# gitouni/Spatial-Temporal-LiDAR-camera-Calibration

Hardware: NVIDIA B200
Metric: extrinsic_cost_evals_per_s (higher is better)
Workload: dtype f64

## Files before the change

### include/stlcalib.h

```cpp
#ifndef STLCALIB_H_
#define STLCALIB_H_

#include <stdint.h>

#ifdef __cplusplus
extern "C" {
#endif

#define STL_ABI_VERSION 2
#define STL_MAX_COVIS 10

typedef enum stl_status {
    STL_OK = 0,
    STL_ERR_INVALID = 1,
    STL_ERR_CUDA = 2,
    STL_ERR_NO_DEVICE = 3,
    STL_ERR_STATE = 4,
    STL_ERR_CAPACITY = 5
} stl_status_t;

typedef struct stl_params {
    double max_pixel_dist;
    double corr_3d_2d_threshold;
    double corr_3d_3d_threshold;
// ... 171 lines not shown

stl_status_t stl_select_keyframes(stl_ctx_t *ctx, const int32_t *kf, int32_t n);

stl_status_t stl_eval_frames(stl_ctx_t *ctx, const double *x, int32_t B, double *out);


stl_status_t stl_debug_corrset(stl_ctx_t *ctx, int32_t b, int32_t kf, uint32_t *kp_idx,
                               uint32_t *pt_idx, int32_t cap, int32_t *n);

stl_status_t stl_debug_align(stl_ctx_t *ctx, int32_t b, int32_t kf, uint32_t *kp_idx,
                             uint32_t *nn_idx, int32_t *n_neigh, int32_t *is_plane, double *dist,
                             uint32_t *knn_idx, int32_t cap, int32_t *n);

stl_status_t stl_debug_frame(stl_ctx_t *ctx, int32_t b, int32_t kf, double out[13]);

stl_status_t stl_knn3d(stl_ctx_t *ctx, int32_t kf, const double *q, int32_t nq, int32_t k,
                       double radius2, uint32_t *out_idx, double *out_d2, int32_t *out_count);

stl_status_t stl_debug_trig(stl_ctx_t *ctx, const double *x, int32_t n, double *acos_out, double *cos_out);


#define STL_STAGE_ASSOC2D 0
#define STL_STAGE_KNN3D 1
#define STL_STAGE_REDUCE 2
#define STL_STAGE_LINEARIZE 3
#define STL_STAGE_BUILD 4
#define STL_STAGE_ASSOC_LM 5
#define STL_STAGE_ALLREDUCE 6
#define STL_STAGE_PLANE_INDEX 7
#define STL_NSTAGES 8
// ... 13 lines not shown
```

### spatial-temporal-lidar-camera-calibration_b200/_abi.py

```python
from __future__ import annotations

import ctypes as C
import os

_HERE = os.path.dirname(os.path.abspath(__file__))

STL_MAX_COVIS = 10
STL_EVAL_NSUMS = 12
STL_LIN_NSUMS = 62
STL_STEP_NSUMS = STL_EVAL_NSUMS + STL_LIN_NSUMS
STL_COMM_ID_BYTES = 128
STL_MAX_PROBLEMS = 256
STL_NSTAGES = 8
STAGE_NAMES = ("assoc2d", "knn3d", "reduce", "linearize", "build", "assoc_lm", "allreduce", "plane_index")

STATUS = {0: "STL_OK", 1: "STL_ERR_INVALID", 2: "STL_ERR_CUDA", 3: "STL_ERR_NO_DEVICE",
          4: "STL_ERR_STATE", 5: "STL_ERR_CAPACITY"}


class StlError(RuntimeError):
    def __init__(self, code: int, msg: str = ""):
        self.code = code
        super().__init__(f"{STATUS.get(code, code)}: {msg}")

# ... 87 lines not shown
        ("width", C.c_int32), ("height", C.c_int32),
        ("fx", C.c_float), ("fy", C.c_float), ("cx", C.c_float), ("cy", C.c_float),
        ("anchored_frac", C.c_double), ("mappoint_frac", C.c_double), ("match_frac", C.c_double),
        ("outlier_frac", C.c_double), ("scale_gt", C.c_double), ("kf_spacing", C.c_double),
        ("max_range", C.c_double), ("elev_top_deg", C.c_double), ("elev_bottom_deg", C.c_double),
        ("x_gt", C.c_double * 7), ("seed", C.c_uint64),
    ]


_vp = C.c_void_p
_dp = C.POINTER(C.c_double)
_u32p = C.POINTER(C.c_uint32)
_i32p = C.POINTER(C.c_int32)
_i64p = C.POINTER(C.c_int64)
_u8p = C.POINTER(C.c_uint8)

CALIB_SYMBOLS = {
    "stl_default_params": (None, [C.POINTER(Params)]),
    "stl_create": (C.c_int, [C.POINTER(Params), C.c_int32, C.POINTER(_vp)]),
    "stl_destroy": (None, [_vp]),
    "stl_last_error": (C.c_char_p, [_vp]),
    "stl_abi_version": (C.c_int32, []),
    "stl_upload_pack": (C.c_int, [_vp, C.POINTER(Pack)]),
    "stl_eval_batch": (C.c_int, [_vp, _dp, C.c_int32, C.POINTER(EvalSums)]),
    "stl_eval_batch_device": (C.c_int, [_vp, _dp, C.c_int32, _vp, _vp]),
    "stl_finalize": (None, [C.POINTER(Params), C.POINTER(EvalSums), C.POINTER(BAErrorOut)]),
    "stl_bbo": (None, [C.POINTER(Params), C.POINTER(BAErrorOut), _dp]),
    "stl_associate": (C.c_int, [_vp, _dp, _i64p]),
    "stl_linearize_batch": (C.c_int, [_vp, _dp, C.c_int32, C.POINTER(LinSums)]),
    "stl_linearize_batch_device": (C.c_int, [_vp, _dp, C.c_int32, _vp, _vp]),
# ... 12 lines not shown
    "stl_step_multi_device": (C.c_int, [_vp, _dp, C.c_int32, _u8p, _vp, _vp]),
    "stl_he_linearize": (C.c_int, [_vp, C.POINTER(HeEdges), _dp, C.c_int32, C.POINTER(LinSums), _dp]),
    "stl_calib_linearize": (C.c_int, [_vp, C.POINTER(CalibEdges), _dp, C.c_int32, C.POINTER(LinSums), _dp]),
    "stl_comm_unique_id": (C.c_int, [C.POINTER(C.c_uint8)]),
    "stl_comm_init": (C.c_int, [_vp, C.POINTER(C.c_uint8), C.c_int32, C.c_int32]),
    "stl_comm_info": (C.c_int, [_vp, _i32p, _i32p]),
    "stl_comm_stats": (C.c_int, [_vp, _i64p]),
    "stl_select_keyframes": (C.c_int, [_vp, _i32p, C.c_int32]),
    "stl_eval_frames": (C.c_int, [_vp, _dp, C.c_int32, _dp]),
    "stl_allow_oversize_keyframes": (C.c_int, [_vp, C.c_int32]),
    "stl_oversize_keyframes": (C.c_int, [_vp, _i32p, C.c_int32, _i32p]),
    "stl_debug_corrset": (C.c_int, [_vp, C.c_int32, C.c_int32, _u32p, _u32p, C.c_int32, _i32p]),
    "stl_debug_align": (C.c_int, [_vp, C.c_int32, C.c_int32, _u32p, _u32p, _i32p, _i32p, _dp, _u32p,
                                  C.c_int32, _i32p]),
    "stl_debug_frame": (C.c_int, [_vp, C.c_int32, C.c_int32, _dp]),
    "stl_debug_trig": (C.c_int, [_vp, _dp, C.c_int32, _dp, _dp]),
    "stl_knn3d": (C.c_int, [_vp, C.c_int32, _dp, C.c_int32, C.c_int32, C.c_double, _u32p, _dp, _i32p]),
    "stl_set_stream": (C.c_int, [_vp, _vp]),
    "stl_set_profiling": (C.c_int, [_vp, C.c_int32]),
    "stl_stage_stats": (C.c_int, [_vp, _dp, _i64p]),
    "stl_work_counters": (C.c_int, [_vp, _dp]),
}

SYNTH_SYMBOLS = {
    "stl_synth_default_cfg": (None, [C.POINTER(SynthCfg)]),
    "stl_synth_create": (_vp, [C.POINTER(SynthCfg)]),
    "stl_synth_pack": (C.POINTER(Pack), [_vp]),
    "stl_synth_x_gt": (_dp, [_vp]),
    "stl_synth_Twl": (_dp, [_vp]),
    "stl_synth_destroy": (None, [_vp]),
# ... 38 lines not shown
```

### spatial-temporal-lidar-camera-calibration_b200/capi.py

```python
from __future__ import annotations

import ctypes as C

import numpy as np

from . import _abi
from .pack import KeyFramePack, default_params

_dp = _abi._dp


def _check(lib, h, code):
    if code != 0:
        msg = lib.stl_last_error(h).decode() if h else ""
        raise _abi.StlError(code, msg)


class Context:

    def __init__(self, params: _abi.Params | None = None, device: int = 0):
        self.lib = _abi.load_calib()
        self.params = params if params is not None else default_params()
        h = C.c_void_p()
        code = self.lib.stl_create(C.byref(self.params), device, C.byref(h))
# ... 294 lines not shown
        knn = np.zeros((cap, 32), np.uint32)
        n = C.c_int32(0)
        _check(self.lib, self.h, self.lib.stl_debug_align(
            self.h, b, kf, kp.ctypes.data_as(_abi._u32p), nn.ctypes.data_as(_abi._u32p), m.ctypes.data_as(_abi._i32p),
            pl.ctypes.data_as(_abi._i32p), d.ctypes.data_as(_dp), knn.ctypes.data_as(_abi._u32p), cap, C.byref(n)))
        k = n.value
        return dict(kp=kp[:k], nn=nn[:k], m=m[:k], is_plane=pl[:k], dist=d[:k], knn=knn[:k])

    def debug_frame(self, b: int, kf: int):
        out = np.zeros(13)
        _check(self.lib, self.h, self.lib.stl_debug_frame(self.h, b, kf, out.ctypes.data_as(_dp)))
        names = ("sum_3d2d", "valid_3d2d", "cnt_3d2d", "sum_he", "cnt_he", "kept", "n_corr", "n_queries",
                 "sum_3d3d", "valid_3d3d", "cnt_3d3d", "valid_pl", "valid_pt")
        return dict(zip(names, out))

    def debug_trig(self, x):
        x = np.ascontiguousarray(x, dtype=np.float64).reshape(-1)
        a, c = np.zeros_like(x), np.zeros_like(x)
        _check(self.lib, self.h, self.lib.stl_debug_trig(self.h, x.ctypes.data_as(_dp), len(x), a.ctypes.data_as(_dp), c.ctypes.data_as(_dp)))
        return a, c

    def knn3d(self, kf: int, q, k: int, radius2: float = 0.0):
        q = np.ascontiguousarray(q, dtype=np.float64).reshape(-1, 3)
        nq = q.shape[0]
        idx = np.zeros((nq, k), np.uint32)
        d2 = np.zeros((nq, k), np.float64)
        cnt = np.zeros(nq, np.int32)
        _check(self.lib, self.h, self.lib.stl_knn3d(self.h, kf, q.ctypes.data_as(_dp), nq, k, radius2,
                                                    idx.ctypes.data_as(_abi._u32p), d2.ctypes.data_as(_dp),
                                                    cnt.ctypes.data_as(_abi._i32p)))
# ... 80 lines not shown
```

### spatial-temporal-lidar-camera-calibration_b200/csrc/capi.cu

```cuda
#include <algorithm>
#include <cfloat>
#include <climits>
#include <cmath>
#include <cstdarg>
#include <cstdio>
#include <cstdlib>
#include <cstring>
#include <mutex>
#include <string>
#include <vector>

#include <nccl.h>

#include "../../include/stlcalib.h"
#include "gprfit.hpp"
#include "hostmath.hpp"
#include "kernels.h"
#include "lm.h"
#include "packlayout.hpp"

using namespace stl;

struct stl_ctx {
    int device = 0;
// ... 82 lines not shown
    }
    return st;
}

#define CK(call)                                                                                          \
    do {                                                                                                  \
        cudaError_t e_ = (call);                                                                          \
        if (e_ != cudaSuccess) return fail(ctx, STL_ERR_CUDA, "%s: %s (%s:%d)", #call, cudaGetErrorString(e_), __FILE__, __LINE__); \
    } while (0)

template <class T> void dfree(T *&p) { if (p) { cudaFree(p); p = nullptr; } }

void free_pack(stl_ctx *c) {
    DevPack &p = c->pk;
    dfree(p.kf); dfree(p.px); dfree(p.py); dfree(p.pz); dfree(p.orig); dfree(p.node_lo); dfree(p.node_hi); dfree(p.adj); dfree(p.adj_cov);
    dfree(p.pl_rec); dfree(p.pl_m);
    dfree(p.k1tab); dfree(p.bitmap); dfree(p.grid_start); dfree(p.grid_kp); dfree(p.kp_xy); dfree(p.kp_xyd); dfree(p.kp_mp); dfree(p.Tcw);
    dfree(p.relpose); dfree(p.covis_valid); dfree(p.covis_uv); dfree(p.he_Tc); dfree(p.he_Tl);
    p = DevPack();
    dfree(c->d_frames); dfree(c->d_ov);
    for (stl_ctx::DevRoute *d : {&c->d_all, &c->d_sel}) { dfree(d->lists); dfree(d->sel); dfree(d->sel_mp); *d = stl_ctx::DevRoute(); }
    c->lay = PackLayout();
    c->route = KfRoute();
    c->has_pack = false;
}
void free_work(stl_ctx *c) {
    DevWork &w = c->wk;
    dfree(w.cand); dfree(w.corr_kp); dfree(w.corr_pt); dfree(w.corr_sp); dfree(w.q_corr); dfree(w.q_kpsp); dfree(w.n_corr); dfree(w.n_q);
    dfree(w.k1_ticket); dfree(w.k1_rec); dfree(w.k1_match); dfree(w.k1_ov_match); dfree(w.k1_surv); dfree(w.k1_cnt); dfree(w.k1_best_d2); dfree(w.k1_best_key);
    dfree(w.frame); dfree(w.align); dfree(w.nn_pos); dfree(w.nn_g2); dfree(w.nb); dfree(w.nbx); dfree(w.nb_m); dfree(w.nb_last); dfree(w.dbg_nn); dfree(w.dbg_m); dfree(w.dbg_plane); dfree(w.dbg_dist); dfree(w.dbg_knn); dfree(w.dbg_stats);
    dfree(w.overflow); dfree(w.k1_clk);
// ... 537 lines not shown
            CK(cudaMemcpy(row.data(), pk.adj + hk[f].node_off * 32, row.size() * 2, cudaMemcpyDeviceToHost));
            cov.resize((size_t)nl);
            CK(cudaMemcpy(cov.data(), pk.adj_cov + hk[f].node_off, cov.size() * 4, cudaMemcpyDeviceToHost));
            for (int l = 0; l < nl; ++l) if (cov[l] >= 0 && cov[l] < 1e30f) { ++partial; cov_sum += std::sqrt((double)cov[l]); }
            for (int l = 0; l < nl; ++l) {
                int c = 0;
                for (int t = 0; t < 32; ++t) c += row[(size_t)l * 32 + t] != 0xffffu;
                ++real; empty += c == 0; entries += c;
            }
        }
        fprintf(stderr, "[stl] leaf adjacency (sampled keyframes): %lld leaves, %.2f%% without a row, %.1f neighbours per row, %.1f%% truncated (mean coverage %.3f m)\n", real,
                100.0 * empty / std::max<long long>(real, 1), (double)entries / std::max<long long>(real - empty, 1),
                100.0 * partial / std::max<long long>(real, 1), cov_sum / std::max<long long>(partial, 1));
    }
    if (ctx->params.plane_index) {
        CK(cudaMalloc(&pk.pl_rec, sizeof(PlaneRec) * npt));
        CK(cudaMalloc(&pk.pl_m, 4 * npt));
        CK(cudaEventRecord(ev0, st));
        for (int f0 = 0; f0 < F;) {
            int f1 = f0 + 1;
            long long pts = hk[f0].n_pad;
            while (f1 < F && pts + hk[f1].n_pad <= (4ll << 20)) pts += hk[f1++].n_pad;
            cudaError_t e = build_plane_index(pk, hk.data(), f0, f1 - f0, ctx->dpr, st, scope.scr);
            if (e != cudaSuccess) return fail(ctx, STL_ERR_CUDA, "plane index: %s", cudaGetErrorString(e));
            f0 = f1;
        }
        CK(cudaEventRecord(ev1, st));
        CK(cudaStreamSynchronize(st));
        float ms = 0;
        CK(cudaEventElapsedTime(&ms, ev0, ev1));
        ctx->stage_ms[STL_STAGE_PLANE_INDEX] += ms;
        ctx->stage_n[STL_STAGE_PLANE_INDEX] += 1;
// ... 85 lines not shown
    if (m <= 0) return STL_OK;
    const long long off = ctx->lay.kf[kf].kp_off;
    if (kp_idx) {
        int nc = 0;
        CK(cudaMemcpy(&nc, ctx->wk.n_corr + kf, 4, cudaMemcpyDeviceToHost));
        std::vector<uint32_t> qc(m), ck(std::max(nc, 1));
        CK(cudaMemcpy(qc.data(), ctx->wk.q_corr + off, 4 * (size_t)m, cudaMemcpyDeviceToHost));
        CK(cudaMemcpy(ck.data(), ctx->wk.corr_kp + off, 4 * (size_t)nc, cudaMemcpyDeviceToHost));
        for (int i = 0; i < m; ++i) kp_idx[i] = ck[qc[i]];
    }
    if (nn_idx) CK(cudaMemcpy(nn_idx, ctx->wk.dbg_nn + off, 4 * (size_t)m, cudaMemcpyDeviceToHost));
    if (n_neigh) CK(cudaMemcpy(n_neigh, ctx->wk.dbg_m + off, 4 * (size_t)m, cudaMemcpyDeviceToHost));
    if (is_plane) CK(cudaMemcpy(is_plane, ctx->wk.dbg_plane + off, 4 * (size_t)m, cudaMemcpyDeviceToHost));
    if (dist) CK(cudaMemcpy(dist, ctx->wk.dbg_dist + off, 8 * (size_t)m, cudaMemcpyDeviceToHost));
    if (knn_idx) CK(cudaMemcpy(knn_idx, ctx->wk.dbg_knn + off * kMaxK, 4 * (size_t)m * kMaxK, cudaMemcpyDeviceToHost));
    return STL_OK;
}

stl_status_t stl_debug_frame(stl_ctx_t *ctx, int32_t b, int32_t kf, double out[13]) {
    if (!ctx || !out) return STL_ERR_INVALID;
    std::lock_guard<std::mutex> lk(ctx->mu);
    CK(cudaSetDevice(ctx->device));
    stl_status_t s = run_debug(ctx, b);
    if (s != STL_OK) return s;
    if (kf < 0 || kf >= ctx->pk.n_kf) return fail(ctx, STL_ERR_INVALID, "keyframe out of range");
    if (!kf_selected(ctx, kf)) { for (int i = 0; i < 13; ++i) out[i] = 0; return STL_OK; }
    FrameRec r;
    CK(cudaMemcpy(&r, ctx->wk.frame + kf, sizeof(r), cudaMemcpyDeviceToHost));
    std::vector<AlignRec> a(ctx->wk.sub);
    CK(cudaMemcpy(a.data(), ctx->wk.align + (size_t)kf * ctx->wk.sub, sizeof(AlignRec) * ctx->wk.sub, cudaMemcpyDeviceToHost));
// ... 645 lines not shown
```

### spatial-temporal-lidar-camera-calibration_b200/csrc/common.cuh

```cuda
#pragma once
#include <cstdint>
#include <cuda_runtime.h>

namespace stl {

constexpr int kLeaf = 32;
constexpr int kPadPts = 128;
constexpr int kBmCell = 2;
constexpr int kGridCell = 8;
constexpr float kFastErrPx = 0.25f;
constexpr int kMaxK = 32;

struct DevKf {
    long long pt_off;
    long long node_off;
    long long kp_off;
    long long bm_off;
    long long grid_off;
    long long mp_off;
    long long tab_off;
    int n_mp;
    int tab_bytes;
    int n_pts, n_pad;
    int n0, n1, n2;
// ... 25 lines not shown
    double s;
    float sf;
    float pad_;
};

struct FrameRec {
    double s2d, v2d, c2d;
    double she, che;
    double kept, ncorr;
    double nq;
};
struct AlignRec {
    double s3d, v3d, c3d, vpl, vpt;
};

struct PlaneRec {
    double nx, ny, nz, reg;
};

struct DevParams {
    double max_pixel_dist2, thr2d, thr3d, radius2, reg_thr, min_diff2;
    double max_3d_dist2, delta2d, delta3d;
    double w0, w1;
    int num_min_corr, k, min_pts, use_plane;
    int use_gpr, plane_index, variant;
    float adj_r;
    double min_diff;
    double gpr_sigma, gpr_l, gpr_noise;
};

__device__ __forceinline__ double dmul(double a, double b) { return __dmul_rn(a, b); }
__device__ __forceinline__ double dadd(double a, double b) { return __dadd_rn(a, b); }
__device__ __forceinline__ double dsub(double a, double b) { return __dsub_rn(a, b); }
// ... 30 lines not shown
```

### spatial-temporal-lidar-camera-calibration_b200/csrc/kernels.h

```cpp
#pragma once
#include <cstddef>
#include <cstdint>
#include <cuda_runtime.h>

#include "common.cuh"
#include "p2p.cuh"

namespace stl {

struct OvKf {
    int f;
    int surv_cap;
    int match_cap;
    int n_bands;
    long long kp_off;
    long long surv_off;
    long long match_off;
};

struct DevPack {
    int n_kf = 0, n_covis = 0;
    long long n_pad_total = 0, n_nodes_total = 0, n_kp_total = 0, n_mp_total = 0;
    DevKf *kf = nullptr;
    float *px = nullptr, *py = nullptr, *pz = nullptr;
    uint32_t *orig = nullptr;
    float4 *node_lo = nullptr, *node_hi = nullptr;
    uint16_t *adj = nullptr;
    float *adj_cov = nullptr;
    PlaneRec *pl_rec = nullptr;
    int *pl_m = nullptr;
    uint8_t *k1tab = nullptr;
    uint32_t *bitmap = nullptr;
    uint32_t *grid_start = nullptr;
    uint32_t *grid_kp = nullptr;
    float2 *kp_xy = nullptr;
    double2 *kp_xyd = nullptr;
    float *kp_mp = nullptr;
    float *Tcw = nullptr;
    float *relpose = nullptr;
    uint8_t *covis_valid = nullptr;
    float2 *covis_uv = nullptr;
    float *he_Tc = nullptr;
    double *he_Tl = nullptr;
    int n_sel = 0;
    const int *sel = nullptr;
// ... 108 lines not shown
```

### spatial-temporal-lidar-camera-calibration_b200/csrc/knn.cuh

```cuda
#pragma once
#include <cfloat>
#include <cmath>

#include "common.cuh"
#include "geom.cuh"
#include "kernels.h"

namespace stl {

constexpr unsigned kFull = 0xffffffffu;

struct ScanView {
    const float *px, *py, *pz;
    const uint32_t *orig;
    const float4 *lo, *hi;
    const uint16_t *adj;
    const float *adj_cov;
    unsigned long long *stats;
    int n0, n1;
};

__device__ __forceinline__ ScanView make_view(const DevPack &pk, const DevKf &K) {
    ScanView v;
    v.px = pk.px + K.pt_off; v.py = pk.py + K.pt_off; v.pz = pk.pz + K.pt_off;
// ... 357 lines not shown
        const V3 d = {x - cx, y - cy, z - cz};
        reg += fabs(dot(d, n));
    }
    out.n = n;
    out.reg = reg / (double)(m - 1);
    if (stable && sqrt(last) < pr.min_diff) out.reg = __longlong_as_double(0x7ff0000000000000ll);
    return out;
}


__device__ __forceinline__ PlaneOut plane_thread(const ScanView &S, const uint32_t *__restrict__ nb, int m, double last, double cx,
                                                 double cy, double cz, const DevParams &pr, const bool stable = false) {
    return plane_fit(NbGather{S, nb}, m, last, cx, cy, cz, pr, stable);
}

__device__ __forceinline__ PlaneOut plane_lookup(const DevPack &pk, const DevKf &K, uint32_t pos) {
    const PlaneRec r = pk.pl_rec[K.pt_off + pos];
    const int mm = pk.pl_m[K.pt_off + pos];
    PlaneOut out;
    out.gates_ok = mm >= 0;
    out.m = mm >= 0 ? mm : -(mm + 1);
    out.n = {r.nx, r.ny, r.nz};
    out.reg = r.reg;
    return out;
}

}
```

### spatial-temporal-lidar-camera-calibration_b200/csrc/knn3d.cu

```cuda
#include <algorithm>
#include <cstdlib>

#include "kernels.h"
#include "knn.cuh"

namespace stl {
namespace {

constexpr int kWarps = 8;
#ifndef STL_KNN_MINB
#define STL_KNN_MINB 8
#endif
constexpr int kPlaneThreads = 128;
#ifndef STL_PLANE_MINB
#define STL_PLANE_MINB 5
#endif

__device__ __forceinline__ void map_point_lidar(const DevPack &pk, const DevKf &K, const DevCand &c, int f, uint32_t kp, double &qx,
                                                double &qy, double &qz) {
    const float *Tcw = pk.Tcw + (long long)f * 12;
    const float *mp = pk.kp_mp + (K.kp_off + kp) * 3;
    const double wx = (double)__fmul_rn(mp[0], c.sf), wy = (double)__fmul_rn(mp[1], c.sf), wz = (double)__fmul_rn(mp[2], c.sf);
    const double cxm = dadd(dot3e((double)Tcw[0], (double)Tcw[1], (double)Tcw[2], wx, wy, wz), dmul((double)Tcw[3], c.s));
    const double cym = dadd(dot3e((double)Tcw[4], (double)Tcw[5], (double)Tcw[6], wx, wy, wz), dmul((double)Tcw[7], c.s));
// ... 20 lines not shown
    __shared__ int ticket;
    if (threadIdx.x == 0) ticket = 0;
    __syncthreads();
    for (;;) {
        const int t0 = next_ticket(&ticket, lane) * batch;
        if ((long long)t0 * sub + j >= nq) break;
        const int qi = (t0 + lane) * sub + j;
        const bool valid = lane < batch && qi < nq;
        double qx = 0, qy = 0, qz = 0, sd = DBL_MAX;
        uint32_t hint = 0, soi = 0xffffffffu, spos = 0xffffffffu;
        float delta = 0.f;
        if (valid) {
            const uint2 ks = wk.q_kpsp[cbase + qi];
            hint = ks.y;
            map_point_lidar(pk, K, c, f, ks.x, qx, qy, qz);
            const double dd = dist3e(qx, qy, qz, (double)S.px[hint], (double)S.py[hint], (double)S.pz[hint]);
            if (dd == dd) { sd = dd; soi = S.orig[hint]; spos = hint; }
            delta = home_box_delta(S, (int)(hint >> 5), qx, qy, qz);
        }
        uint32_t out_pos = 0xffffffffu;
        float out_g2 = 0.f;
        unsigned todo = __ballot_sync(kFull, valid);
        while (todo) {
            const int src = __ffs(todo) - 1;
            todo &= todo - 1;
            const double x = __shfl_sync(kFull, qx, src), y = __shfl_sync(kFull, qy, src), z = __shfl_sync(kFull, qz, src);
            const uint32_t h = __shfl_sync(kFull, hint, src);
            Sink1 nn;
            nn.d = __shfl_sync(kFull, sd, src);
            nn.oi = __shfl_sync(kFull, soi, src);
            nn.pos = __shfl_sync(kFull, spos, src);
// ... 14 lines not shown
        if (lm_pos != nullptr && b == 0) {
            double lx = 0, ly = 0, lz = 0, nn_d = DBL_MAX;
            uint32_t nn_p = 0xffffffffu;
            bool need = false;
            if (valid) {
                const float *Tcw = pk.Tcw + (long long)f * 12;
                const float *mp = pk.kp_mp + (K.kp_off + wk.q_kpsp[cbase + qi].x) * 3;
                const double ma = (double)mp[0], mb = (double)mp[1], mc = (double)mp[2];
                const double Mx = dadd(dot3e((double)Tcw[0], (double)Tcw[1], (double)Tcw[2], ma, mb, mc), (double)Tcw[3]);
                const double My = dadd(dot3e((double)Tcw[4], (double)Tcw[5], (double)Tcw[6], ma, mb, mc), (double)Tcw[7]);
                const double Mz = dadd(dot3e((double)Tcw[8], (double)Tcw[9], (double)Tcw[10], ma, mb, mc), (double)Tcw[11]);
                xform(c.Ri, c.ti, dmul(Mx, c.s), dmul(My, c.s), dmul(Mz, c.s), lx, ly, lz);
                need = true;
                if (out_pos != 0xffffffffu) {
                    const double move = sqrt(dist3e(qx, qy, qz, lx, ly, lz)) * (1.0 + 1e-9) + 1e-12;
                    const double dh = dist3e(lx, ly, lz, (double)S.px[out_pos], (double)S.py[out_pos], (double)S.pz[out_pos]);
                    const double reach = (double)__fsqrt_rd(out_g2) - move;
                    if (reach > 0.0 && reach * reach > dh * (1.0 + 1e-6) + 1e-18) { need = false; nn_p = out_pos; nn_d = dh; }
                }
            }
            unsigned todo2 = __ballot_sync(kFull, need);
            while (todo2) {
                const int src = __ffs(todo2) - 1;
                todo2 &= todo2 - 1;
                const double x = __shfl_sync(kFull, lx, src), y = __shfl_sync(kFull, ly, src), z = __shfl_sync(kFull, lz, src);
                uint32_t h = __shfl_sync(kFull, out_pos, src);
                if (h == 0xffffffffu) h = __shfl_sync(kFull, hint, src);
                Sink1 nn;
                nn_near_leaf(S, pr.adj_r, (int)(h >> 5), x, y, z, nn, lane, h);
                if (lane == src) { nn_p = nn.pos; nn_d = nn.d; }
            }
// ... 14 lines not shown
k_plane_dist(const DevPack pk, const DevWork wk, const DevParams pr, const int B, const int debug) {
    const int sub = wk.sub;
    const int j = blockIdx.x % sub;
    const int bf = blockIdx.x / sub;
    const int fi = bf / B, f = sel_kf(pk, fi), b = bf - fi * B;
    const long long rec = (long long)b * pk.n_kf + f;
    const int nq = wk.n_q[rec];
    double s3d = 0, v3d = 0, c3d = 0, vpl = 0, vpt = 0;
    if (nq > 0) {
        const DevKf K = pk.kf[f];
        const DevCand &c = wk.cand[b];
        const ScanView S = make_view(pk, K);
        const long long cbase = (long long)b * pk.n_kp_total + K.kp_off;
        const long long qbase = (long long)b * pk.n_mp_total + K.mp_off;
        for (int qi = j * kPlaneThreads + threadIdx.x; qi < nq; qi += sub * kPlaneThreads) {
            const uint32_t kp = wk.corr_kp[cbase + wk.q_corr[cbase + qi]];
            double qx, qy, qz;
            map_point_lidar(pk, K, c, f, kp, qx, qy, qz);
            const uint32_t np = wk.nn_pos[qbase + qi];
            const double nx = (double)S.px[np], ny = (double)S.py[np], nz = (double)S.pz[np];
            const double dx = dsub(nx, qx), dy = dsub(ny, qy), dz = dsub(nz, qz);
            double dist = sqrt(dot3e(dx, dy, dz, dx, dy, dz));
            int is_plane = 0, m = 0;
            if (pr.use_plane) {
                const PlaneOut po = pr.plane_index ? plane_lookup(pk, K, np)
                                                   : plane_fit(NbCoords{wk.nbx + qbase + qi, wk.nbx_stride}, wk.nb_m[qbase + qi], wk.nb_last[qbase + qi], nx, ny, nz, pr, pr.variant == 1);
                m = po.m;
                if (po.gates_ok && !(po.reg > pr.reg_thr)) {
                    is_plane = 1;
                    dist = fabs(dot3e(dx, dy, dz, po.n.x, po.n.y, po.n.z));
                }
            }
            if (dist < pr.thr3d) {
                s3d += dist; v3d += 1.0;
                if (is_plane) vpl += 1.0; else vpt += 1.0;
            }
            c3d += 1.0;
            if (debug) {
                const long long o = K.kp_off + qi;
                wk.dbg_nn[o] = S.orig[np];
                wk.dbg_m[o] = m;
// ... 49 lines not shown
        SinkK kn(pr.k, pr.radius2);
        knn_around_point(S, (uint32_t)p, kn, lane);
        const long long o = K.pt_off - first_pt + p;
        nb[o * kMaxK + lane] = lane < kn.count ? kn.kpos : 0xffffffffu;
        const double last = __shfl_sync(kFull, kn.kd, kn.count > 0 ? kn.count - 1 : 0);
        if (lane == 0) { nb_m[o] = kn.count; nb_last[o] = last; }
    }
}

__global__ void __launch_bounds__(kPlaneThreads)
k_index_plane(const DevPack pk, const int kf_begin, const DevParams pr, const long long first_pt, const uint32_t *__restrict__ nb,
              const int *__restrict__ nb_m, const double *__restrict__ nb_last) {
    const DevKf K = pk.kf[kf_begin + blockIdx.y];
    const ScanView S = make_view(pk, K);
    for (int p = blockIdx.x * kPlaneThreads + threadIdx.x; p < K.n_pad; p += gridDim.x * kPlaneThreads) {
        PlaneRec r = {0.0, 0.0, 0.0, 0.0};
        int mm = -1;
        if (p < K.n_pts) {
            const long long o = K.pt_off - first_pt + p;
            const PlaneOut po = plane_thread(S, nb + o * kMaxK, nb_m[o], nb_last[o], (double)S.px[p], (double)S.py[p], (double)S.pz[p], pr, pr.variant == 1);
            r.nx = po.n.x; r.ny = po.n.y; r.nz = po.n.z; r.reg = po.reg;
            mm = po.gates_ok ? po.m : -(po.m + 1);
        }
        pk.pl_rec[K.pt_off + p] = r;
        pk.pl_m[K.pt_off + p] = mm;
    }
}

}

cudaError_t build_plane_index(const DevPack &pk, const DevKf *h_kf, int kf_begin, int nkf, const DevParams &pr, cudaStream_t st,
                              BuildScratch &scr) {
    const long long first = h_kf[kf_begin].pt_off;
    const long long npts = h_kf[kf_begin + nkf - 1].pt_off + h_kf[kf_begin + nkf - 1].n_pad - first;
    if (npts <= 0) return cudaSuccess;
    int max_pts = 0;
    for (int f = 0; f < nkf; ++f) max_pts = max_pts > h_kf[kf_begin + f].n_pad ? max_pts : h_kf[kf_begin + f].n_pad;
    cudaError_t e = scr.need(2, 4 * (size_t)npts * kMaxK);
    if (e == cudaSuccess) e = scr.need(4, 4 * (size_t)npts);
    if (e == cudaSuccess) e = scr.need(3, 8 * (size_t)npts);
// ... 46 lines not shown
```

### spatial-temporal-lidar-camera-calibration_b200/csrc/lm.cu

```cuda
#include <cub/cub.cuh>

#include "../../include/stlcalib.h"
#include "dual.cuh"
#include "gprfit.hpp"
#include "knn.cuh"
#include "lm.h"

namespace stl {
namespace {

constexpr int kWarps = 8;
#ifndef STL_LM_MINB
#define STL_LM_MINB 6
#endif
constexpr int kLinVals = 41;
constexpr int kGprWarps = 1;
constexpr int kLinThreads = 128;


__device__ __forceinline__ void lm_lane(const DevPack &pk, DevWork &wk, LmState &lm, bool arg0 = true) {
    const int2 am = arg0 && blockIdx.y == 0 ? lm.lane0 : lm.amap[blockIdx.y];
    const long long nk = pk.n_kp_total, F = pk.n_kf, nm = lm.n_slots;
    const long long wc = am.x, wq = wc * nm;
    wk.cand += wc;
// ... 72 lines not shown
k_lm_plane_a(const DevPack pk, DevWork wk, const DevParams pr, LmState lm) {
    lm_lane(pk, wk, lm);
    const int j = blockIdx.x % lm.sub, f = sel_kf(pk, blockIdx.x / lm.sub);
    int nq;
    if (!lm_frame_active(wk, pr, f, nq)) return;
    __shared__ int cnt[2];
    if (threadIdx.x < 2) cnt[threadIdx.x] = 0;
    __syncthreads();
    const DevKf K = pk.kf[f];
    const ScanView S = make_view(pk, K);
    const bool from_index = pr.plane_index && !pr.use_gpr;
    const int C = pk.n_covis;
    for (int qi = j * blockDim.x + threadIdx.x; qi < nq; qi += lm.sub * blockDim.x) {
        const long long slot = K.mp_off + qi;
        lm.stage[slot] = 0;
        const uint32_t ci = wk.q_corr[K.kp_off + qi];
        const uint32_t kp = wk.corr_kp[K.kp_off + ci], sp = wk.corr_sp[K.kp_off + ci];
        int m = 0;
        if (from_index) {
            bool any = false;
            for (int s = 0; s < C; ++s) any = any || (pk.covis_valid[f * C + s] && !isnan(pk.covis_uv[(K.kp_off + kp) * C + s].x));
            if (!any) continue;
        } else {
            m = wk.nb_m[slot];
            if (m < 0) continue;
        }
        const double cx = (double)S.px[sp], cy = (double)S.py[sp], cz = (double)S.pz[sp];
        const PlaneOut po = from_index ? plane_lookup(pk, K, sp)
                                       : plane_fit(NbCoords{wk.nbx + slot, wk.nbx_stride}, m, wk.nb_last[slot], cx, cy, cz, pr);
        if (!po.gates_ok) continue;
        const long long cs = slot;
        lm.slot_kf[cs] = f;
        lm.slot_kp[cs] = kp;
        double *pa = lm.plane_a + slot * 4;
        pa[0] = po.n.x; pa[1] = po.n.y; pa[2] = po.n.z; pa[3] = po.reg;
        if (po.reg < pr.reg_thr) {
            double *g = lm.geo2d + cs * 6;
            g[0] = cx; g[1] = cy; g[2] = cz; g[3] = po.n.x; g[4] = po.n.y; g[5] = po.n.z;
            lm.flag2d[cs] = 1;
            atomicAdd(&cnt[0], 1);
        } else if (pr.use_gpr) {
            for (int t = 0; t < kMaxK; ++t) lm.gpr_nb[slot * kMaxK + t] = wk.nb[slot * kMaxK + t];
            lm.gpr_m[slot] = po.m;
            lm.flagG[cs] = 1;
// ... 36 lines not shown
            sp = ks.y;
            double Mx, My, Mz;
            lm_map_point(pk, K, f, kp, Mx, My, Mz);
            xform(c0.Ri, c0.ti, dmul(Mx, c0.s), dmul(My, c0.s), dmul(Mz, c0.s), qx, qy, qz);
            hint = nn_hint ? nn_hint[slot] : sp;
            if (hint == 0xffffffffu) hint = sp;
            if (nn_hint && nn_g2 && nn_hint[slot] != 0xffffffffu) {
                const float *mp = pk.kp_mp + (K.kp_off + kp) * 3;
                const double wx = (double)__fmul_rn(mp[0], c0.sf), wy = (double)__fmul_rn(mp[1], c0.sf), wz = (double)__fmul_rn(mp[2], c0.sf);
                const double ex = dadd(dot3e((double)Tcw[0], (double)Tcw[1], (double)Tcw[2], wx, wy, wz), dmul((double)Tcw[3], c0.s));
                const double ey = dadd(dot3e((double)Tcw[4], (double)Tcw[5], (double)Tcw[6], wx, wy, wz), dmul((double)Tcw[7], c0.s));
                const double ez = dadd(dot3e((double)Tcw[8], (double)Tcw[9], (double)Tcw[10], wx, wy, wz), dmul((double)Tcw[11], c0.s));
                double ox, oy, oz;
                xform(c0.Ri, c0.ti, ex, ey, ez, ox, oy, oz);
                const double move = sqrt(dist3e(ox, oy, oz, qx, qy, qz)) * (1.0 + 1e-9) + 1e-12;
                const double dh = dist3e(qx, qy, qz, (double)S.px[hint], (double)S.py[hint], (double)S.pz[hint]);
                const double reach = (double)__fsqrt_rd(nn_g2[slot]) - move;
                if (reach > 0.0 && reach * reach > dh * (1.0 + 1e-6) + 1e-18) { settled = true; nn_pos = hint; nn_d = dh; }
            }
        }
        unsigned todo = __ballot_sync(kFull, valid && !settled);
        while (todo) {
            const int src = __ffs(todo) - 1;
            todo &= todo - 1;
            const double sx = __shfl_sync(kFull, qx, src), sy = __shfl_sync(kFull, qy, src), sz = __shfl_sync(kFull, qz, src);
            const uint32_t sh = __shfl_sync(kFull, hint, src);
            Sink1 nn;
            nn_near_leaf(S, pr.adj_r, (int)(sh >> 5), sx, sy, sz, nn, lane, sh);
            if (lane == src) { nn_pos = nn.pos; nn_d = nn.d; }
        }
        bool want_knn = false;
// ... 11 lines not shown
        while (kn_todo) {
            const int src = __ffs(kn_todo) - 1;
            kn_todo &= kn_todo - 1;
            const uint32_t p = __shfl_sync(kFull, nn_pos, src);
            const long long sl = K.mp_off + ((long long)(base + src) * lm.sub + j);
            SinkK kn(pr.k, pr.radius2);
            knn_around_point(S, p, kn, lane);
            lm.nbb[sl * kMaxK + lane] = lane < kn.count ? kn.kpos : 0xffffffffu;
            store_nb_coords(lm.nbbx, lm.nbbx_stride, sl, S, lane, kn.count, kn.kpos);
            const double last = __shfl_sync(kFull, kn.kd, kn.count > 0 ? kn.count - 1 : 0);
            if (lane == 0) { lm.nbb_m[sl] = kn.count; lm.nbb_last[sl] = last; }
        }
    }
}

__device__ __forceinline__ bool block3d_geometry(const DevPack &pk, const DevParams &pr, const LmState &lm, long long slot, int f, uint32_t kp,
                                                 double g[9], int &type) {
    if (lm.stage[slot] != 1) return false;
    const uint32_t np = lm.nnb_pos[slot];
    if (np == 0xffffffffu) return false;
    const DevKf &K = pk.kf[f];
    const float *sx = pk.px + K.pt_off, *sy = pk.py + K.pt_off, *sz = pk.pz + K.pt_off;
    const double nx = (double)sx[np], ny = (double)sy[np], nz = (double)sz[np];
    bool gates_ok, state;
    double n3[3];
    const int m = lm.nbb_m[slot];
    if (m == -2) {
        const double *pa = lm.plane_a + slot * 4;
        gates_ok = true; n3[0] = pa[0]; n3[1] = pa[1]; n3[2] = pa[2];
        state = pa[3] < pr.reg_thr;
    } else {
        const PlaneOut p2 = m == -3 ? plane_lookup(pk, K, np) : plane_fit(NbCoords{lm.nbbx + slot, lm.nbbx_stride}, m, lm.nbb_last[slot], nx, ny, nz, pr);
        gates_ok = p2.gates_ok; n3[0] = p2.n.x; n3[1] = p2.n.y; n3[2] = p2.n.z;
        state = p2.gates_ok && p2.reg < pr.reg_thr;
    }
    lm_map_point(pk, K, f, kp, g[0], g[1], g[2]);
    g[3] = nx; g[4] = ny; g[5] = nz;
    g[6] = gates_ok ? n3[0] : 0.0; g[7] = gates_ok ? n3[1] : 0.0; g[8] = gates_ok ? n3[2] : 1.0;
    type = state ? 2 : 1;
    return true;
}

__global__ void __launch_bounds__(128)
k_lm_plane_b(const DevPack pk, DevWork wk, const DevParams pr, LmState lm) {
    lm_lane(pk, wk, lm, false);
    const int j = blockIdx.x % lm.sub, f = sel_kf(pk, blockIdx.x / lm.sub);
    int nq;
    if (!lm_frame_active(wk, pr, f, nq)) return;
    const DevKf K = pk.kf[f];
    __shared__ int cnt[2];
    if (threadIdx.x < 2) cnt[threadIdx.x] = 0;
    __syncthreads();
    for (int qi = j * blockDim.x + threadIdx.x; qi < nq; qi += lm.sub * blockDim.x) {
        const long long slot = K.mp_off + qi;
        if (lm.stage[slot] != 1) continue;
        if (lm.nnb_pos[slot] == 0xffffffffu) continue;
        const uint32_t ci = wk.q_corr[K.kp_off + qi];
        const uint32_t kp = wk.corr_kp[K.kp_off + ci];
        double g9[9];
        int type;
        if (!block3d_geometry(pk, pr, lm, slot, f, kp, g9, type)) continue;
        double *g = lm.geo3d + slot * 9;
#pragma unroll
        for (int i = 0; i < 9; ++i) g[i] = g9[i];
        lm.type3d[slot] = (uint8_t)type;
        lm.flag3d[slot] = 1;
        atomicAdd(&cnt[0], 1);
        if (type == 1) atomicAdd(&cnt[1], 1);
    }
    __syncthreads();
    if (threadIdx.x < 2 && cnt[threadIdx.x] > 0) atomicAdd(lm.d_counts + 1 + threadIdx.x, cnt[threadIdx.x]);
}

struct Acc {
    double v[kLinVals];
};
// ... 831 lines not shown
```

Baseline: 1075.

## Pack point coords and plane records into one aligned SurfRec array

```diff
diff --git a/include/stlcalib.h b/include/stlcalib.h
--- a/include/stlcalib.h
+++ b/include/stlcalib.h
@@ -209,6 +209,9 @@
 
 stl_status_t stl_debug_frame(stl_ctx_t *ctx, int32_t b, int32_t kf, double out[13]);
 
+stl_status_t stl_debug_surf(stl_ctx_t *ctx, int32_t kf, float *xyz, int32_t *m, double *plane, uint32_t *orig,
+                            int32_t cap, int32_t *n);
+
 stl_status_t stl_knn3d(stl_ctx_t *ctx, int32_t kf, const double *q, int32_t nq, int32_t k,
                        double radius2, uint32_t *out_idx, double *out_d2, int32_t *out_count);
 
diff --git a/spatial-temporal-lidar-camera-calibration_b200/_abi.py b/spatial-temporal-lidar-camera-calibration_b200/_abi.py
--- a/spatial-temporal-lidar-camera-calibration_b200/_abi.py
+++ b/spatial-temporal-lidar-camera-calibration_b200/_abi.py
@@ -125,6 +125,7 @@
 _i32p = C.POINTER(C.c_int32)
 _i64p = C.POINTER(C.c_int64)
 _u8p = C.POINTER(C.c_uint8)
+_fp = C.POINTER(C.c_float)
 
 CALIB_SYMBOLS = {
     "stl_default_params": (None, [C.POINTER(Params)]),
@@ -167,6 +168,7 @@
     "stl_debug_align": (C.c_int, [_vp, C.c_int32, C.c_int32, _u32p, _u32p, _i32p, _i32p, _dp, _u32p,
                                   C.c_int32, _i32p]),
     "stl_debug_frame": (C.c_int, [_vp, C.c_int32, C.c_int32, _dp]),
+    "stl_debug_surf": (C.c_int, [_vp, C.c_int32, _fp, _i32p, _dp, _u32p, C.c_int32, _i32p]),
     "stl_debug_trig": (C.c_int, [_vp, _dp, C.c_int32, _dp, _dp]),
     "stl_knn3d": (C.c_int, [_vp, C.c_int32, _dp, C.c_int32, C.c_int32, C.c_double, _u32p, _dp, _i32p]),
     "stl_set_stream": (C.c_int, [_vp, _vp]),
diff --git a/spatial-temporal-lidar-camera-calibration_b200/capi.py b/spatial-temporal-lidar-camera-calibration_b200/capi.py
--- a/spatial-temporal-lidar-camera-calibration_b200/capi.py
+++ b/spatial-temporal-lidar-camera-calibration_b200/capi.py
@@ -332,6 +332,19 @@
                  "sum_3d3d", "valid_3d3d", "cnt_3d3d", "valid_pl", "valid_pt")
         return dict(zip(names, out))
 
+    def debug_surf(self, kf: int):
+        cap = int(self.pack.scan_offset[kf + 1] - self.pack.scan_offset[kf]) if self.pack is not None else 1 << 20
+        cap = max(cap, 1)
+        xyz = np.zeros((cap, 3), np.float32)
+        m = np.zeros(cap, np.int32)
+        plane = np.zeros((cap, 4), np.float64)
+        orig = np.zeros(cap, np.uint32)
+        n = C.c_int32(0)
+        _check(self.lib, self.h, self.lib.stl_debug_surf(self.h, kf, xyz.ctypes.data_as(_abi._fp), m.ctypes.data_as(_abi._i32p),
+                                                         plane.ctypes.data_as(_dp), orig.ctypes.data_as(_abi._u32p), cap, C.byref(n)))
+        k = min(n.value, cap)
+        return dict(xyz=xyz[:k], m=m[:k], plane=plane[:k], orig=orig[:k])
+
     def debug_trig(self, x):
         x = np.ascontiguousarray(x, dtype=np.float64).reshape(-1)
         a, c = np.zeros_like(x), np.zeros_like(x)
diff --git a/spatial-temporal-lidar-camera-calibration_b200/csrc/capi.cu b/spatial-temporal-lidar-camera-calibration_b200/csrc/capi.cu
--- a/spatial-temporal-lidar-camera-calibration_b200/csrc/capi.cu
+++ b/spatial-temporal-lidar-camera-calibration_b200/csrc/capi.cu
@@ -120,7 +120,7 @@
 void free_pack(stl_ctx *c) {
     DevPack &p = c->pk;
     dfree(p.kf); dfree(p.px); dfree(p.py); dfree(p.pz); dfree(p.orig); dfree(p.node_lo); dfree(p.node_hi); dfree(p.adj); dfree(p.adj_cov);
-    dfree(p.pl_rec); dfree(p.pl_m);
+    dfree(p.surf);
     dfree(p.k1tab); dfree(p.bitmap); dfree(p.grid_start); dfree(p.grid_kp); dfree(p.kp_xy); dfree(p.kp_xyd); dfree(p.kp_mp); dfree(p.Tcw);
     dfree(p.relpose); dfree(p.covis_valid); dfree(p.covis_uv); dfree(p.he_Tc); dfree(p.he_Tl);
     p = DevPack();
@@ -688,8 +688,7 @@
                 100.0 * partial / std::max<long long>(real, 1), cov_sum / std::max<long long>(partial, 1));
     }
     if (ctx->params.plane_index) {
-        CK(cudaMalloc(&pk.pl_rec, sizeof(PlaneRec) * npt));
-        CK(cudaMalloc(&pk.pl_m, 4 * npt));
+        CK(cudaMalloc(&pk.surf, sizeof(SurfRec) * npt));
         CK(cudaEventRecord(ev0, st));
         for (int f0 = 0; f0 < F;) {
             int f1 = f0 + 1;
@@ -805,6 +804,28 @@
     if (is_plane) CK(cudaMemcpy(is_plane, ctx->wk.dbg_plane + off, 4 * (size_t)m, cudaMemcpyDeviceToHost));
     if (dist) CK(cudaMemcpy(dist, ctx->wk.dbg_dist + off, 8 * (size_t)m, cudaMemcpyDeviceToHost));
     if (knn_idx) CK(cudaMemcpy(knn_idx, ctx->wk.dbg_knn + off * kMaxK, 4 * (size_t)m * kMaxK, cudaMemcpyDeviceToHost));
+    return STL_OK;
+}
+
+stl_status_t stl_debug_surf(stl_ctx_t *ctx, int32_t kf, float *xyz, int32_t *m, double *plane, uint32_t *orig, int32_t cap, int32_t *n) {
+    if (!ctx || !n) return STL_ERR_INVALID;
+    std::lock_guard<std::mutex> lk(ctx->mu);
+    CK(cudaSetDevice(ctx->device));
+    if (!ctx->has_pack) return fail(ctx, STL_ERR_STATE, "stl_upload_pack has not been called");
+    if (!ctx->pk.surf) return fail(ctx, STL_ERR_STATE, "the pack was uploaded without the plane index");
+    if (kf < 0 || kf >= ctx->pk.n_kf) return fail(ctx, STL_ERR_INVALID, "keyframe out of range");
+    const DevKf &K = ctx->lay.kf[kf];
+    *n = K.n_pts;
+    const int cnt = std::min(K.n_pts, cap);
+    if (cnt <= 0) return STL_OK;
+    std::vector<SurfRec> r(cnt);
+    CK(cudaMemcpy(r.data(), ctx->pk.surf + K.pt_off, sizeof(SurfRec) * (size_t)cnt, cudaMemcpyDeviceToHost));
+    if (orig) CK(cudaMemcpy(orig, ctx->pk.orig + K.pt_off, 4 * (size_t)cnt, cudaMemcpyDeviceToHost));
+    for (int i = 0; i < cnt; ++i) {
+        if (xyz) { xyz[3 * i] = r[i].x; xyz[3 * i + 1] = r[i].y; xyz[3 * i + 2] = r[i].z; }
+        if (m) m[i] = r[i].m;
+        if (plane) { plane[4 * i] = r[i].nx; plane[4 * i + 1] = r[i].ny; plane[4 * i + 2] = r[i].nz; plane[4 * i + 3] = r[i].reg; }
+    }
     return STL_OK;
 }
 
diff --git a/spatial-temporal-lidar-camera-calibration_b200/csrc/common.cuh b/spatial-temporal-lidar-camera-calibration_b200/csrc/common.cuh
--- a/spatial-temporal-lidar-camera-calibration_b200/csrc/common.cuh
+++ b/spatial-temporal-lidar-camera-calibration_b200/csrc/common.cuh
@@ -63,9 +63,12 @@
     double s3d, v3d, c3d, vpl, vpt;
 };
 
-struct PlaneRec {
+struct alignas(16) SurfRec {
+    float x, y, z;
+    int m;
     double nx, ny, nz, reg;
 };
+static_assert(sizeof(SurfRec) == 48, "SurfRec is three 16-byte words");
 
 struct DevParams {
     double max_pixel_dist2, thr2d, thr3d, radius2, reg_thr, min_diff2;
diff --git a/spatial-temporal-lidar-camera-calibration_b200/csrc/kernels.h b/spatial-temporal-lidar-camera-calibration_b200/csrc/kernels.h
--- a/spatial-temporal-lidar-camera-calibration_b200/csrc/kernels.h
+++ b/spatial-temporal-lidar-camera-calibration_b200/csrc/kernels.h
@@ -27,8 +27,7 @@
     float4 *node_lo = nullptr, *node_hi = nullptr;
     uint16_t *adj = nullptr;
     float *adj_cov = nullptr;
-    PlaneRec *pl_rec = nullptr;
-    int *pl_m = nullptr;
+    SurfRec *surf = nullptr;
     uint8_t *k1tab = nullptr;
     uint32_t *bitmap = nullptr;
     uint32_t *grid_start = nullptr;
diff --git a/spatial-temporal-lidar-camera-calibration_b200/csrc/knn.cuh b/spatial-temporal-lidar-camera-calibration_b200/csrc/knn.cuh
--- a/spatial-temporal-lidar-camera-calibration_b200/csrc/knn.cuh
+++ b/spatial-temporal-lidar-camera-calibration_b200/csrc/knn.cuh
@@ -395,15 +395,23 @@
     return plane_fit(NbGather{S, nb}, m, last, cx, cy, cz, pr, stable);
 }
 
-__device__ __forceinline__ PlaneOut plane_lookup(const DevPack &pk, const DevKf &K, uint32_t pos) {
-    const PlaneRec r = pk.pl_rec[K.pt_off + pos];
-    const int mm = pk.pl_m[K.pt_off + pos];
+__device__ __forceinline__ PlaneOut plane_lookup(const DevPack &pk, const DevKf &K, uint32_t pos, double &x, double &y, double &z) {
+    const float4 *r = reinterpret_cast<const float4 *>(pk.surf + K.pt_off + pos);
+    const float4 p = r[0];
+    const double2 n01 = reinterpret_cast<const double2 *>(r)[1], n2r = reinterpret_cast<const double2 *>(r)[2];
+    x = (double)p.x; y = (double)p.y; z = (double)p.z;
+    const int mm = __float_as_int(p.w);
     PlaneOut out;
     out.gates_ok = mm >= 0;
     out.m = mm >= 0 ? mm : -(mm + 1);
-    out.n = {r.nx, r.ny, r.nz};
-    out.reg = r.reg;
+    out.n = {n01.x, n01.y, n2r.x};
+    out.reg = n2r.y;
     return out;
 }
 
-}
+__device__ __forceinline__ void surf_point(const DevPack &pk, const DevKf &K, uint32_t pos, double &x, double &y, double &z) {
+    const float4 p = *reinterpret_cast<const float4 *>(pk.surf + K.pt_off + pos);
+    x = (double)p.x; y = (double)p.y; z = (double)p.z;
+}
+
+}
diff --git a/spatial-temporal-lidar-camera-calibration_b200/csrc/knn3d.cu b/spatial-temporal-lidar-camera-calibration_b200/csrc/knn3d.cu
--- a/spatial-temporal-lidar-camera-calibration_b200/csrc/knn3d.cu
+++ b/spatial-temporal-lidar-camera-calibration_b200/csrc/knn3d.cu
@@ -58,7 +58,10 @@
             const uint2 ks = wk.q_kpsp[cbase + qi];
             hint = ks.y;
             map_point_lidar(pk, K, c, f, ks.x, qx, qy, qz);
-            const double dd = dist3e(qx, qy, qz, (double)S.px[hint], (double)S.py[hint], (double)S.pz[hint]);
+            double hx, hy, hz;
+            if (pr.plane_index) surf_point(pk, K, hint, hx, hy, hz);
+            else { hx = (double)S.px[hint]; hy = (double)S.py[hint]; hz = (double)S.pz[hint]; }
+            const double dd = dist3e(qx, qy, qz, hx, hy, hz);
             if (dd == dd) { sd = dd; soi = S.orig[hint]; spos = hint; }
             delta = home_box_delta(S, (int)(hint >> 5), qx, qy, qz);
         }
@@ -103,7 +106,9 @@
                 need = true;
                 if (out_pos != 0xffffffffu) {
                     const double move = sqrt(dist3e(qx, qy, qz, lx, ly, lz)) * (1.0 + 1e-9) + 1e-12;
-                    const double dh = dist3e(lx, ly, lz, (double)S.px[out_pos], (double)S.py[out_pos], (double)S.pz[out_pos]);
+                    double ox, oy, oz;
+                    surf_point(pk, K, out_pos, ox, oy, oz);
+                    const double dh = dist3e(lx, ly, lz, ox, oy, oz);
                     const double reach = (double)__fsqrt_rd(out_g2) - move;
                     if (reach > 0.0 && reach * reach > dh * (1.0 + 1e-6) + 1e-18) { need = false; nn_p = out_pos; nn_d = dh; }
                 }
@@ -148,17 +153,23 @@
         const long long cbase = (long long)b * pk.n_kp_total + K.kp_off;
         const long long qbase = (long long)b * pk.n_mp_total + K.mp_off;
         for (int qi = j * kPlaneThreads + threadIdx.x; qi < nq; qi += sub * kPlaneThreads) {
-            const uint32_t kp = wk.corr_kp[cbase + wk.q_corr[cbase + qi]];
+            const uint32_t kp = wk.q_kpsp[cbase + qi].x;
             double qx, qy, qz;
             map_point_lidar(pk, K, c, f, kp, qx, qy, qz);
             const uint32_t np = wk.nn_pos[qbase + qi];
-            const double nx = (double)S.px[np], ny = (double)S.py[np], nz = (double)S.pz[np];
+            double nx, ny, nz;
+            PlaneOut po;
+            if (pr.plane_index) {
+                po = plane_lookup(pk, K, np, nx, ny, nz);
+            } else {
+                nx = (double)S.px[np]; ny = (double)S.py[np]; nz = (double)S.pz[np];
+            }
             const double dx = dsub(nx, qx), dy = dsub(ny, qy), dz = dsub(nz, qz);
             double dist = sqrt(dot3e(dx, dy, dz, dx, dy, dz));
             int is_plane = 0, m = 0;
             if (pr.use_plane) {
-                const PlaneOut po = pr.plane_index ? plane_lookup(pk, K, np)
-                                                   : plane_fit(NbCoords{wk.nbx + qbase + qi, wk.nbx_stride}, wk.nb_m[qbase + qi], wk.nb_last[qbase + qi], nx, ny, nz, pr, pr.variant == 1);
+                if (!pr.plane_index)
+                    po = plane_fit(NbCoords{wk.nbx + qbase + qi, wk.nbx_stride}, wk.nb_m[qbase + qi], wk.nb_last[qbase + qi], nx, ny, nz, pr, pr.variant == 1);
                 m = po.m;
                 if (po.gates_ok && !(po.reg > pr.reg_thr)) {
                     is_plane = 1;
@@ -238,16 +249,14 @@
     const DevKf K = pk.kf[kf_begin + blockIdx.y];
     const ScanView S = make_view(pk, K);
     for (int p = blockIdx.x * kPlaneThreads + threadIdx.x; p < K.n_pad; p += gridDim.x * kPlaneThreads) {
-        PlaneRec r = {0.0, 0.0, 0.0, 0.0};
-        int mm = -1;
+        SurfRec r = {S.px[p], S.py[p], S.pz[p], -1, 0.0, 0.0, 0.0, 0.0};
         if (p < K.n_pts) {
             const long long o = K.pt_off - first_pt + p;
-            const PlaneOut po = plane_thread(S, nb + o * kMaxK, nb_m[o], nb_last[o], (double)S.px[p], (double)S.py[p], (double)S.pz[p], pr, pr.variant == 1);
+            const PlaneOut po = plane_thread(S, nb + o * kMaxK, nb_m[o], nb_last[o], (double)r.x, (double)r.y, (double)r.z, pr, pr.variant == 1);
             r.nx = po.n.x; r.ny = po.n.y; r.nz = po.n.z; r.reg = po.reg;
-            mm = po.gates_ok ? po.m : -(po.m + 1);
-        }
-        pk.pl_rec[K.pt_off + p] = r;
-        pk.pl_m[K.pt_off + p] = mm;
+            r.m = po.gates_ok ? po.m : -(po.m + 1);
+        }
+        pk.surf[K.pt_off + p] = r;
     }
 }
 
diff --git a/spatial-temporal-lidar-camera-calibration_b200/csrc/lm.cu b/spatial-temporal-lidar-camera-calibration_b200/csrc/lm.cu
--- a/spatial-temporal-lidar-camera-calibration_b200/csrc/lm.cu
+++ b/spatial-temporal-lidar-camera-calibration_b200/csrc/lm.cu
@@ -110,20 +110,22 @@
     for (int qi = j * blockDim.x + threadIdx.x; qi < nq; qi += lm.sub * blockDim.x) {
         const long long slot = K.mp_off + qi;
         lm.stage[slot] = 0;
-        const uint32_t ci = wk.q_corr[K.kp_off + qi];
-        const uint32_t kp = wk.corr_kp[K.kp_off + ci], sp = wk.corr_sp[K.kp_off + ci];
+        const uint2 ks = wk.q_kpsp[K.kp_off + qi];
+        const uint32_t kp = ks.x, sp = ks.y;
         int m = 0;
+        double cx, cy, cz;
+        PlaneOut po;
         if (from_index) {
+            po = plane_lookup(pk, K, sp, cx, cy, cz);
             bool any = false;
             for (int s = 0; s < C; ++s) any = any || (pk.covis_valid[f * C + s] && !isnan(pk.covis_uv[(K.kp_off + kp) * C + s].x));
             if (!any) continue;
         } else {
             m = wk.nb_m[slot];
             if (m < 0) continue;
-        }
-        const double cx = (double)S.px[sp], cy = (double)S.py[sp], cz = (double)S.pz[sp];
-        const PlaneOut po = from_index ? plane_lookup(pk, K, sp)
-                                       : plane_fit(NbCoords{wk.nbx + slot, wk.nbx_stride}, m, wk.nb_last[slot], cx, cy, cz, pr);
+            cx = (double)S.px[sp]; cy = (double)S.py[sp]; cz = (double)S.pz[sp];
+            po = plane_fit(NbCoords{wk.nbx + slot, wk.nbx_stride}, m, wk.nb_last[slot], cx, cy, cz, pr);
+        }
         if (!po.gates_ok) continue;
         const long long cs = slot;
         lm.slot_kf[cs] = f;
@@ -190,7 +192,10 @@
                 double ox, oy, oz;
                 xform(c0.Ri, c0.ti, ex, ey, ez, ox, oy, oz);
                 const double move = sqrt(dist3e(ox, oy, oz, qx, qy, qz)) * (1.0 + 1e-9) + 1e-12;
-                const double dh = dist3e(qx, qy, qz, (double)S.px[hint], (double)S.py[hint], (double)S.pz[hint]);
+                double hx, hy, hz;
+                if (pr.plane_index) surf_point(pk, K, hint, hx, hy, hz);
+                else { hx = (double)S.px[hint]; hy = (double)S.py[hint]; hz = (double)S.pz[hint]; }
+                const double dh = dist3e(qx, qy, qz, hx, hy, hz);
                 const double reach = (double)__fsqrt_rd(nn_g2[slot]) - move;
                 if (reach > 0.0 && reach * reach > dh * (1.0 + 1e-6) + 1e-18) { settled = true; nn_pos = hint; nn_d = dh; }
             }
@@ -232,31 +237,32 @@
     }
 }
 
-__device__ __forceinline__ bool block3d_geometry(const DevPack &pk, const DevParams &pr, const LmState &lm, long long slot, int f, uint32_t kp,
-                                                 double g[9], int &type) {
-    if (lm.stage[slot] != 1) return false;
-    const uint32_t np = lm.nnb_pos[slot];
-    if (np == 0xffffffffu) return false;
-    const DevKf &K = pk.kf[f];
-    const float *sx = pk.px + K.pt_off, *sy = pk.py + K.pt_off, *sz = pk.pz + K.pt_off;
-    const double nx = (double)sx[np], ny = (double)sy[np], nz = (double)sz[np];
+__device__ __forceinline__ void block3d_geometry(const DevPack &pk, const DevParams &pr, const LmState &lm, const DevKf &K, long long slot,
+                                                 int f, uint32_t kp, uint32_t np, int m, double g[9], int &type) {
+    lm_map_point(pk, K, f, kp, g[0], g[1], g[2]);
+    double nx, ny, nz;
     bool gates_ok, state;
     double n3[3];
-    const int m = lm.nbb_m[slot];
+    PlaneOut p2;
+    if (m == -3) {
+        p2 = plane_lookup(pk, K, np, nx, ny, nz);
+    } else if (pr.plane_index) {
+        surf_point(pk, K, np, nx, ny, nz);
+    } else {
+        nx = (double)pk.px[K.pt_off + np]; ny = (double)pk.py[K.pt_off + np]; nz = (double)pk.pz[K.pt_off + np];
+    }
     if (m == -2) {
         const double *pa = lm.plane_a + slot * 4;
         gates_ok = true; n3[0] = pa[0]; n3[1] = pa[1]; n3[2] = pa[2];
         state = pa[3] < pr.reg_thr;
     } else {
-        const PlaneOut p2 = m == -3 ? plane_lookup(pk, K, np) : plane_fit(NbCoords{lm.nbbx + slot, lm.nbbx_stride}, m, lm.nbb_last[slot], nx, ny, nz, pr);
+        if (m != -3) p2 = plane_fit(NbCoords{lm.nbbx + slot, lm.nbbx_stride}, m, lm.nbb_last[slot], nx, ny, nz, pr);
         gates_ok = p2.gates_ok; n3[0] = p2.n.x; n3[1] = p2.n.y; n3[2] = p2.n.z;
         state = p2.gates_ok && p2.reg < pr.reg_thr;
     }
-    lm_map_point(pk, K, f, kp, g[0], g[1], g[2]);
     g[3] = nx; g[4] = ny; g[5] = nz;
     g[6] = gates_ok ? n3[0] : 0.0; g[7] = gates_ok ? n3[1] : 0.0; g[8] = gates_ok ? n3[2] : 1.0;
     type = state ? 2 : 1;
-    return true;
 }
 
 __global__ void __launch_bounds__(128)
@@ -271,13 +277,14 @@
     __syncthreads();
     for (int qi = j * blockDim.x + threadIdx.x; qi < nq; qi += lm.sub * blockDim.x) {
         const long long slot = K.mp_off + qi;
-        if (lm.stage[slot] != 1) continue;
-        if (lm.nnb_pos[slot] == 0xffffffffu) continue;
-        const uint32_t ci = wk.q_corr[K.kp_off + qi];
-        const uint32_t kp = wk.corr_kp[K.kp_off + ci];
+        const uint8_t stage = lm.stage[slot];
+        const uint32_t np = lm.nnb_pos[slot];
+        const int m = lm.nbb_m[slot];
+        const uint32_t kp = wk.q_kpsp[K.kp_off + qi].x;
+        if (stage != 1 || np == 0xffffffffu) continue;
         double g9[9];
         int type;
-        if (!block3d_geometry(pk, pr, lm, slot, f, kp, g9, type)) continue;
+        block3d_geometry(pk, pr, lm, K, slot, f, kp, np, m, g9, type);
         double *g = lm.geo3d + slot * 9;
 #pragma unroll
         for (int i = 0; i < 9; ++i) g[i] = g9[i];
```

After: 1112, median of 6. +3.5%, better.
